# bbc/turingcodec

Hardware: AMD Instinct MI355X
Metric: encoded fps (havoc hot path, primitive-batch throughput: one picture's primitive calls per frame as whole-frame batches; (higher is better)
Workload: dtype u8; 1 GPU; 1920x1080 8-bit 4:2:0 random-access QP32 speed=medium B-frame, MEASURED call mix of the reference encoder on this clip generator (profiles/r04_reference_call_mi; calls_per_frame=3944815, launches_per_frame=49, pictures_in_flight=2, parallelism=single GPU

## Files before the change

turingcodec_amd/csrc/common.h:

```cpp
#pragma once

#include <hip/hip_runtime.h>
#include <stdint.h>

#include "../../include/havoc_mi355x.h"

namespace havoc_gpu {

constexpr int kWave = 64;

typedef uint32_t __attribute__((aligned(1))) u32u;
typedef uint32_t __attribute__((ext_vector_type(2), aligned(1))) u32x2u;
typedef uint32_t __attribute__((ext_vector_type(4), aligned(1))) u32x4u;
typedef uint32_t __attribute__((ext_vector_type(2))) u32x2;
typedef uint32_t __attribute__((ext_vector_type(4))) u32x4;
typedef short __attribute__((ext_vector_type(2))) s16x2;
typedef unsigned short __attribute__((ext_vector_type(2))) u16x2;

__device__ __forceinline__ uint32_t ld4(const void *p) { return *reinterpret_cast<const u32u *>(p); }
__device__ __forceinline__ u32x2 ld8(const void *p)
{
    u32x2u v = *reinterpret_cast<const u32x2u *>(p);
    return u32x2{v.x, v.y};
}
__device__ __forceinline__ u32x4 ld16(const void *p)
{
    u32x4u v = *reinterpret_cast<const u32x4u *>(p);
    return u32x4{v.x, v.y, v.z, v.w};
}
__device__ __forceinline__ void st4(void *p, uint32_t v) { *reinterpret_cast<u32u *>(p) = v; }
__device__ __forceinline__ void st8(void *p, u32x2 v) { *reinterpret_cast<u32x2u *>(p) = u32x2u{v.x, v.y}; }
__device__ __forceinline__ void st16(void *p, u32x4 v) { *reinterpret_cast<u32x4u *>(p) = u32x4u{v.x, v.y, v.z, v.w}; }

__device__ __forceinline__ int wave_sum(int v)
{
    v += __builtin_amdgcn_update_dpp(0, v, 0x111, 0xf, 0xf, true);
    v += __builtin_amdgcn_update_dpp(0, v, 0x112, 0xf, 0xf, true);
    v += __builtin_amdgcn_update_dpp(0, v, 0x114, 0xf, 0xe, true);
    v += __builtin_amdgcn_update_dpp(0, v, 0x118, 0xf, 0xc, true);
    v += __builtin_amdgcn_update_dpp(0, v, 0x142, 0xa, 0xf, true);
    v += __builtin_amdgcn_update_dpp(0, v, 0x143, 0xc, 0xf, true);
    return __builtin_amdgcn_readlane(v, 63);
}

__device__ __forceinline__ int row16_sum(int v)
{
    v += __builtin_amdgcn_update_dpp(0, v, 0x111, 0xf, 0xf, true);
    v += __builtin_amdgcn_update_dpp(0, v, 0x112, 0xf, 0xf, true);
    v += __builtin_amdgcn_update_dpp(0, v, 0x114, 0xf, 0xe, true);
    v += __builtin_amdgcn_update_dpp(0, v, 0x118, 0xf, 0xc, true);
    return v;
}

template <int G>
__device__ __forceinline__ int group_sum(int v)
{
#pragma unroll
    for (int o = 1; o < G; o <<= 1) v += __shfl_xor(v, o, kWave);
    return v;
}

__device__ __forceinline__ int xcd_block(int b, int nb)
{
    const int q = nb >> 3, r = nb & 7;
    const int x = b & 7, i = b >> 3;
    return x * q + min(x, r) + i;
}

__device__ __forceinline__ int clip3(int lo, int hi, int v) { return min(max(v, lo), hi); }

struct FastDiv
{
    uint32_t inv;
    int d;
    __device__ __forceinline__ explicit FastDiv(int d_) : d(d_)
    {
        const uint32_t ud = (uint32_t)d_;
        const uint32_t i0 = (uint32_t)(1048576.0f * __builtin_amdgcn_rcpf((float)d_)) - 1u;
        const uint32_t r = (1u << 20) - i0 * ud;
        inv = i0 + (r > 0u) + (r > ud) + (r > 2u * ud);
    }
    __device__ __forceinline__ int div(int i) const { return d == 1 ? i : (int)(((uint32_t)i * inv) >> 20); }
};


template <int N>
__device__ __forceinline__ void wht_inplace(int (&v)[N])
{
#pragma unroll
    for (int len = 1; len < N; len <<= 1)
#pragma unroll
        for (int i = 0; i < N; i += len << 1)
#pragma unroll
            for (int k = i; k < i + len; ++k)
            {
                const int a = v[k], b = v[k + len];
                v[k] = a + b;
                v[k + len] = a - b;
            }
}

template <int CTRL>
__device__ __forceinline__ int dpp_mov(int v)
{
    return __builtin_amdgcn_update_dpp(0, v, CTRL, 0xf, 0xf, true);
}

constexpr int kDppXor1 = 0xB1;
constexpr int kDppXor3 = 0x1B;
constexpr int kDppHalfMirror = 0x141;

template <int S, int TS>
__device__ __forceinline__ int satd_rows(int (&d)[TS], int r)
{
    wht_inplace<TS>(d);
    if (TS == 8)
    {
        const int s4 = (r & 4) ? -1 : 1;
#pragma unroll
        for (int k = 0; k < TS; ++k) d[k] = dpp_mov<kDppHalfMirror>(d[k]) + s4 * d[k];
    }
    const int s2 = (r & 2) ? -1 : 1, s1 = (r & 1) ? -1 : 1;
#pragma unroll
    for (int k = 0; k < TS; ++k) d[k] = dpp_mov<kDppXor3>(d[k]) + s2 * d[k];
    int sum = 0;
#pragma unroll
    for (int k = 0; k < TS; ++k) sum += abs(dpp_mov<kDppXor1>(d[k]) + s1 * d[k]);
    sum += dpp_mov<kDppXor1>(sum);
    sum += dpp_mov<kDppXor3>(sum);
    if (TS == 8) sum += dpp_mov<kDppHalfMirror>(sum);
    sum = (sum + TS / 4) / (TS / 2);
    if (S == 2) sum >>= 2;
    return r == 0 ? sum : 0;
}

__device__ __forceinline__ uint32_t pk_add(uint32_t a, uint32_t b)
{
    return __builtin_bit_cast(uint32_t, __builtin_bit_cast(s16x2, a) + __builtin_bit_cast(s16x2, b));
}
__device__ __forceinline__ uint32_t pk_sub(uint32_t a, uint32_t b)
{
    return __builtin_bit_cast(uint32_t, __builtin_bit_cast(s16x2, a) - __builtin_bit_cast(s16x2, b));
}
__device__ __forceinline__ uint32_t pk_bfly(uint32_t v)
{
    const u16x2 t = __builtin_bit_cast(u16x2, __builtin_amdgcn_alignbit(v, v, 16));
    const u16x2 sgn = {1, 0xffff};
    return __builtin_bit_cast(uint32_t, __builtin_bit_cast(u16x2, v) * sgn + t);
}
__device__ __forceinline__ uint32_t pk_abs_acc(uint32_t v, uint32_t acc)
{
    return __builtin_amdgcn_sad_u16(v ^ 0x80008000u, 0x80008000u, acc);
}

template <int TS>
__device__ __forceinline__ int satd_rows_pk(uint32_t (&p)[TS / 2], int r)
{
#pragma unroll
    for (int k = 0; k < TS / 2; ++k) p[k] = pk_bfly(p[k]);
#pragma unroll
    for (int len = 1; len < TS / 2; len <<= 1)
#pragma unroll
        for (int i = 0; i < TS / 2; i += len << 1)
#pragma unroll
            for (int k = i; k < i + len; ++k)
            {
                const uint32_t a = p[k], b = p[k + len];
                p[k] = pk_add(a, b);
                p[k + len] = pk_sub(a, b);
            }
    const s16x2 one = {1, 1}, neg = {-1, -1};
    if (TS == 8)
    {
        const s16x2 s4 = (r & 4) ? neg : one;
#pragma unroll
        for (int k = 0; k < TS / 2; ++k)
            p[k] = __builtin_bit_cast(uint32_t, __builtin_bit_cast(s16x2, p[k]) * s4 + __builtin_bit_cast(s16x2, (uint32_t)dpp_mov<kDppHalfMirror>((int)p[k])));
    }
    const s16x2 s2 = (r & 2) ? neg : one, s1 = (r & 1) ? neg : one;
#pragma unroll
    for (int k = 0; k < TS / 2; ++k)
        p[k] = __builtin_bit_cast(uint32_t, __builtin_bit_cast(s16x2, p[k]) * s2 + __builtin_bit_cast(s16x2, (uint32_t)dpp_mov<kDppXor3>((int)p[k])));
    uint32_t sum = 0;
#pragma unroll
    for (int k = 0; k < TS / 2; ++k)
        sum = pk_abs_acc(__builtin_bit_cast(uint32_t, __builtin_bit_cast(s16x2, p[k]) * s1 + __builtin_bit_cast(s16x2, (uint32_t)dpp_mov<kDppXor1>((int)p[k]))), sum);
    int t = (int)sum;
    t += dpp_mov<kDppXor1>(t);
    t += dpp_mov<kDppXor3>(t);
    if (TS == 8) t += dpp_mov<kDppHalfMirror>(t);
    t = (t + TS / 4) / (TS / 2);
    return r == 0 ? t : 0;
}

__device__ __forceinline__ int satd_tile8_pk(uint32_t (&d)[8][4])
{
#pragma unroll
    for (int r = 0; r < 8; ++r)
    {
        const uint32_t a0 = pk_add(d[r][0], d[r][1]), a1 = pk_sub(d[r][0], d[r][1]), a2 = pk_add(d[r][2], d[r][3]), a3 = pk_sub(d[r][2], d[r][3]);
        d[r][0] = pk_add(a0, a2); d[r][2] = pk_sub(a0, a2);
        d[r][1] = pk_add(a1, a3); d[r][3] = pk_sub(a1, a3);
    }
#pragma unroll
    for (int len = 1; len < 8; len <<= 1)
#pragma unroll
        for (int i = 0; i < 8; i += len << 1)
#pragma unroll
            for (int r = i; r < i + len; ++r)
#pragma unroll
                for (int k = 0; k < 4; ++k)
                {
                    const uint32_t a = d[r][k], b = d[r + len][k];
                    d[r][k] = pk_add(a, b);
                    d[r + len][k] = pk_sub(a, b);
                }
    uint32_t sum = 0;
#pragma unroll
    for (int r = 0; r < 8; ++r)
#pragma unroll
        for (int k = 0; k < 4; ++k) sum = pk_abs_acc(pk_bfly(d[r][k]), sum);
    return (int)((sum + 2) >> 2);
}

__device__ __forceinline__ int satd_tile8_pk16(uint32_t (&d)[8][4])
{
#pragma unroll
    for (int r = 0; r < 8; ++r)
    {
        const uint32_t a0 = pk_add(d[r][0], d[r][1]), a1 = pk_sub(d[r][0], d[r][1]), a2 = pk_add(d[r][2], d[r][3]), a3 = pk_sub(d[r][2], d[r][3]);
        d[r][0] = pk_add(a0, a2); d[r][2] = pk_sub(a0, a2);
        d[r][1] = pk_add(a1, a3); d[r][3] = pk_sub(a1, a3);
    }
#pragma unroll
    for (int len = 1; len < 8; len <<= 1)
#pragma unroll
        for (int i = 0; i < 8; i += len << 1)
#pragma unroll
            for (int r = i; r < i + len; ++r)
#pragma unroll
                for (int k = 0; k < 4; ++k)
                {
                    const uint32_t a = d[r][k], b = d[r + len][k];
                    d[r][k] = pk_add(a, b);
                    d[r + len][k] = pk_sub(a, b);
                }
    uint32_t X = 0, Y = 0;
#pragma unroll
    for (int r = 0; r < 8; ++r)
#pragma unroll
        for (int k = 0; k < 4; ++k)
        {
            const s16x2 v = __builtin_bit_cast(s16x2, d[r][k]);
            const uint32_t mag = __builtin_bit_cast(uint32_t, __builtin_elementwise_max(v, (s16x2){0, 0} - v));
            X = __builtin_amdgcn_sad_u16(mag, 0u, X);
            Y = __builtin_amdgcn_sad_u16(mag, __builtin_amdgcn_alignbit(mag, mag, 16), Y);
        }
    const uint32_t sum = X + (Y >> 1);
    return (int)(((sum + 2) >> 2) >> 2);
}


__host__ __device__ constexpr int angle_of(int mode)
{
    const int d = mode < 18 ? mode - 10 : mode - 26;
    const int mag = (int)((0x2069544d245080ull >> (6 * (d < 0 ? -d : d))) & 63);
    return (mode < 18) == (d < 0) ? mag : -mag;
}
__host__ __device__ constexpr int inv_angle_of(int mode)
{
    const int i = (mode < 18 ? mode - 10 : 26 - mode) - 1;
    const unsigned long long lo = 4096ull | (1638ull << 13) | (910ull << 26) | (630ull << 39);
    const unsigned long long hi = 482ull | (390ull << 13) | (315ull << 26) | (256ull << 39);
    return -(int)(((i < 4 ? lo : hi) >> (13 * (i & 3))) & 0x1fff);
}


typedef uint32_t __attribute__((ext_vector_type(4), aligned(2))) u32x4h;
typedef uint32_t __attribute__((ext_vector_type(2), aligned(2))) u32x2h;

template <int TS>
__device__ __forceinline__ void ld_pairs(const uint16_t *q, uint32_t (&o)[TS / 2])
{
    if constexpr (TS == 8)
    {
        const u32x4h v = *reinterpret_cast<const u32x4h *>(q);
        o[0] = v.x; o[1] = v.y; o[2] = v.z; o[3] = v.w;
    }
    else
    {
        const u32x2h v = *reinterpret_cast<const u32x2h *>(q);
        o[0] = v.x; o[1] = v.y;
    }
}

__device__ __forceinline__ uint32_t pk_mad_u16(uint32_t a, uint32_t b, uint32_t c)
{
    uint32_t d;
    asm("v_pk_mad_u16 %0, %1, %2, %3" : "=v"(d) : "v"(a), "v"(b), "v"(c));
    return d;
}
__device__ __forceinline__ uint32_t pk_lerp(uint32_t a, uint32_t b, uint32_t w0, uint32_t w1)
{
    const u16x2 five = {5, 5};
    const uint32_t t = pk_mad_u16(b, w1, pk_mad_u16(a, w0, 0x00100010u));
    return __builtin_bit_cast(uint32_t, __builtin_bit_cast(u16x2, t) >> five);
}

template <int S> struct Sample;
template <> struct Sample<1> { typedef uint8_t T; };
template <> struct Sample<2> { typedef uint16_t T; };

template <int S>
__device__ __forceinline__ uint32_t ssd_dword(uint32_t a, uint32_t b, uint32_t acc)
{
    if (S == 1)
    {
        acc = __builtin_amdgcn_udot4(a, a, acc, false);
        acc = __builtin_amdgcn_udot4(b, b, acc, false);
        const uint32_t ab = __builtin_amdgcn_udot4(a, b, 0u, false);
        return acc - 2u * ab;
    }
    const u16x2 va = __builtin_bit_cast(u16x2, a), vb = __builtin_bit_cast(u16x2, b);
    acc = __builtin_amdgcn_udot2(va, va, acc, false);
    acc = __builtin_amdgcn_udot2(vb, vb, acc, false);
    const uint32_t ab = __builtin_amdgcn_udot2(va, vb, 0u, false);
    return acc - 2u * ab;
}

}
```

turingcodec_amd/csrc/kernels_tu_fused.hip:

```cpp
#include "common.h"

#include <cstdlib>
#include "transform_basis.h"
#include "launch.h"
#include "rdoq_work.h"

namespace havoc_gpu {

template <int S, int N>
__device__ __forceinline__ void load_sample_row(const char *p, uint32_t (&row)[N / 2])
{
    if (S == 1)
    {
        uint32_t b[N / 4];
        if (N == 4) b[0] = ld4(p);
        else if (N == 8)
        {
            const u32x2 v = ld8(p);
            b[0] = v.x; b[1] = v.y;
        }
        else
        {
#pragma unroll
            for (int q = 0; q < N / 16; ++q)
            {
                const u32x4 v = ld16(p + 16 * q);
                b[4 * q] = v.x; b[4 * q + 1] = v.y; b[4 * q + 2] = v.z; b[4 * q + 3] = v.w;
            }
        }
#pragma unroll
        for (int q = 0; q < N / 4; ++q)
        {
            row[2 * q] = __builtin_amdgcn_perm(0u, b[q], 0x0c010c00u);
            row[2 * q + 1] = __builtin_amdgcn_perm(0u, b[q], 0x0c030c02u);
        }
    }
    else
    {
        if (N == 4)
        {
            const u32x2 v = ld8(p);
            row[0] = v.x; row[1] = v.y;
        }
        else
        {
#pragma unroll
            for (int q = 0; q < N / 8; ++q)
            {
                const u32x4 v = ld16(p + 16 * q);
                row[4 * q] = v.x; row[4 * q + 1] = v.y; row[4 * q + 2] = v.z; row[4 * q + 3] = v.w;
            }
        }
    }
}

template <int N>
__device__ __forceinline__ void store_staged_row(int16_t *g, const int16_t *p)
{
    if constexpr (N == 4) st8(g, *reinterpret_cast<const u32x2 *>(p));
    else st16(g, *reinterpret_cast<const u32x4 *>(p));
}

template <int S, int LOG2, int TR, bool SCAN = false>
__global__ __launch_bounds__(64) void k_tu_forward(int16_t *__restrict__ coeffs, const char *__restrict__ src, long stride_src,
                                                   const char *__restrict__ pred, long stride_pred, const int32_t *__restrict__ jobs, int njobs,
                                                   int bitDepth, const RdoqJob *__restrict__ rjobs = nullptr, int16_t *__restrict__ levels = nullptr,
                                                   RdoqWork *__restrict__ work = nullptr)
{
    constexpr int N = 1 << LOG2, TPW = 64 / N, LS = N + 2;
    __shared__ __attribute__((aligned(16))) int16_t lds[TPW][N * LS];
    const int t = threadIdx.x / N, r = threadIdx.x % N;
    const int job = xcd_block(blockIdx.x, gridDim.x) * TPW + t;
    const bool live = job < njobs;
    const int32_t *j = jobs + (long)(live ? job : 0) * 4;
    const int shift1 = LOG2 - 1 + bitDepth - 8, shift2 = LOG2 + 6;

    uint32_t row[N / 2], prow[N / 2];
    load_sample_row<S, N>(src + ((long)j[1] + (long)r * stride_src) * S, row);
    load_sample_row<S, N>(pred + ((long)j[2] + (long)r * stride_pred) * S, prow);
#pragma unroll
    for (int p = 0; p < N / 2; ++p) row[p] = pk_sub(row[p], prow[p]);
    int o[N];
    basis_times_row<N, TR, false, true>(row, 1 << (shift1 - 1), o);
#pragma unroll
    for (int k = 0; k < N; ++k) lds[t][k * LS + r] = (int16_t)(o[k] >> shift1);
    __syncthreads();
#pragma unroll
    for (int p = 0; p < N / 2; ++p) row[p] = *reinterpret_cast<const uint32_t *>(&lds[t][r * LS + 2 * p]);
    basis_times_row<N, TR, false>(row, 1 << (shift2 - 1), o);
    if (SCAN)
    {
        constexpr int GW = N / 4;
        const RdoqJob rj = rjobs[live ? job : 0];
        uint32_t thr[3];
        rdoqThresholds(rj.quant_scale, rj.quant_shift, thr);
        uint32_t lo = 0, hi = 0;
        uint64_t mask[3] = {0, 0, 0};
#pragma unroll
        for (int gy = 0; gy < GW; ++gy)
        {
            uint32_t big = 0;
#pragma unroll
            for (int k = 4 * gy; k < 4 * gy + 4; ++k)
            {
                const int c = (int16_t)(o[k] >> shift2);
                big = max(big, (uint32_t)abs(c));
                const uint32_t sq = (uint32_t)(c * c);
                lo += sq & 0xffffu;
                hi += sq >> 16;
            }
            big = max(big, (uint32_t)__shfl_xor((int)big, 1, kWave));
            big = max(big, (uint32_t)__shfl_xor((int)big, 2, kWave));
#pragma unroll
            for (int m = 0; m < 3; ++m)
            {
                const uint64_t b = __ballot(live && (r & 3) == 0 && big >= thr[m]) >> (t * N);
                uint32_t f = 0;
#pragma unroll
                for (int gx = 0; gx < GW; ++gx) f |= (uint32_t)((b >> (4 * gx)) & 1) << gx;
                mask[m] |= (uint64_t)f << (gy * GW);
            }
        }
        const int slo = group_sum<N>((int)lo), shi = group_sum<N>((int)hi);
        if (live)
        {
            int16_t *z = levels + rj.dst_off + r * N;
#pragma unroll
            for (int q = 0; q < N / 4; ++q) st8(z + 4 * q, u32x2{0, 0});
            if (r == 0)
            {
                RdoqInfo *info = reinterpret_cast<RdoqInfo *>(reinterpret_cast<char *>(work) + rdoqInfoOffset());
                RdoqInfo v;
                v.mask = mask[0];
                v.mask2 = mask[1];
                v.mask3 = mask[2];
                v.sumSq = ((int64_t)shi << 16) + slo;
                info[job] = v;
            }
        }
    }
    if constexpr (N <= 8)
    {
        __syncthreads();
#pragma unroll
        for (int k = 0; k < N; ++k) lds[t][k * N + r] = (int16_t)(o[k] >> shift2);
        __syncthreads();
        if (!live) return;
        store_staged_row<N>(coeffs + j[0] + r * N, &lds[t][r * N]);
    }
    else
    {
        if (!live) return;
        int16_t *c = coeffs + j[0] + r;
#pragma unroll
        for (int k = 0; k < N; ++k) c[k * N] = (int16_t)(o[k] >> shift2);
    }
}

template <int S, int LOG2, int TR>
__global__ __launch_bounds__(64) void k_tu_reconstruct(char *rec, long stride_rec, const char *pred, long stride_pred, const char *__restrict__ src,
                                                       long stride_src, const int16_t *__restrict__ levels, const int32_t *__restrict__ jobs,
                                                       int njobs, int bitDepth, int scale, int shift, uint32_t *__restrict__ ssd)
{
    typedef typename Sample<S>::T T;
    constexpr int N = 1 << LOG2, TPW = 64 / N, LS = N + 2;
    __shared__ int16_t lds[TPW][N * LS];
    const int t = threadIdx.x / N, r = threadIdx.x % N;
    const int job = xcd_block(blockIdx.x, gridDim.x) * TPW + t;
    const bool live = job < njobs;
    const int32_t *j = jobs + (long)(live ? job : 0) * 4;
    const int shift2 = 20 - bitDepth;
    const int dqadd = 1 << (shift - 1);

    const int16_t *c = levels + j[0] + r;
    uint32_t col[N / 2];
#pragma unroll
    for (int p = 0; p < N / 2; ++p)
    {
        const int lo = clip3(-32768, 32767, ((int)c[(2 * p) * N] * scale + dqadd) >> shift);
        const int hi = clip3(-32768, 32767, ((int)c[(2 * p + 1) * N] * scale + dqadd) >> shift);
        col[p] = ((uint32_t)lo & 0xffffu) | ((uint32_t)hi << 16);
    }
    int o[N];
    basis_times_row<N, TR, true>(col, 1 << 6, o);
#pragma unroll
    for (int k = 0; k < N; ++k) lds[t][k * LS + r] = (int16_t)clip3(-32768, 32767, o[k] >> 7);
    __syncthreads();
#pragma unroll
    for (int p = 0; p < N / 2; ++p) col[p] = *reinterpret_cast<const uint32_t *>(&lds[t][r * LS + 2 * p]);
    basis_times_row<N, TR, true>(col, 1 << (shift2 - 1), o);

    const int maxv = (1 << bitDepth) - 1;
    uint32_t prow[N / 2], srow[N / 2];
    load_sample_row<S, N>(pred + ((long)j[2] + (long)r * stride_pred) * S, prow);
    load_sample_row<S, N>(src + ((long)j[1] + (long)r * stride_src) * S, srow);
    uint32_t acc = 0;
    int v[N];
#pragma unroll
    for (int k = 0; k < N; ++k)
    {
        const int res = clip3(-32768, 32767, o[k] >> shift2);
        const int pk = (k & 1) ? (int)(prow[k >> 1] >> 16) : (int)(prow[k >> 1] & 0xffff);
        const int sk = (k & 1) ? (int)(srow[k >> 1] >> 16) : (int)(srow[k >> 1] & 0xffff);
        v[k] = clip3(0, maxv, pk + res);
        const int d = sk - v[k];
        acc += (uint32_t)(d * d);
    }
    if (live)
    {
        T *q = reinterpret_cast<T *>(rec) + j[3] + (long)r * stride_rec;
        if (S == 1)
        {
#pragma unroll
            for (int k = 0; k < N; k += 4) st4(q + k, (uint32_t)v[k] | ((uint32_t)v[k + 1] << 8) | ((uint32_t)v[k + 2] << 16) | ((uint32_t)v[k + 3] << 24));
        }
        else
        {
#pragma unroll
            for (int k = 0; k < N; k += 2) st4(q + k, (uint32_t)v[k] | ((uint32_t)v[k + 1] << 16));
        }
    }
    uint32_t tot = (uint32_t)group_sum<N>((int)acc);
    if (S == 2) tot >>= 4;
    if (live && r == 0) ssd[job] = tot;
}

template <int S, int LOG2>
__global__ __launch_bounds__(64) void k_intra_measure(int16_t *__restrict__ coeffs, int16_t *__restrict__ coeffsDct, int32_t *__restrict__ satd, char *__restrict__ rec0,
                                                      uint32_t *__restrict__ ssd0, const char *__restrict__ src, long stride_src, const char *__restrict__ pred,
                                                      long stride_pred, const int32_t *__restrict__ jobs, int njobs, int bitDepth, int withSatd)
{
    typedef typename Sample<S>::T T;
    constexpr int N = 1 << LOG2, TPW = 64 / N, LS = N + 2, TS = N >= 8 ? 8 : 4, TX = N / TS, TILES = TX * TX;
    __shared__ int16_t lds[TPW][N * LS];
    const int t = threadIdx.x / N, r = threadIdx.x % N;
    const int job = blockIdx.x * TPW + t;
    const bool live = job < njobs;
    const int32_t *j = jobs + (long)(live ? job : 0) * 4;
    const int shift1 = LOG2 - 1 + bitDepth - 8, shift2 = LOG2 + 6;

    uint32_t row[N / 2], prow[N / 2];
    load_sample_row<S, N>(src + ((long)j[1] + (long)r * stride_src) * S, row);
    load_sample_row<S, N>(pred + ((long)j[2] + (long)r * stride_pred) * S, prow);
    if (live)
    {
        const int maxv = (1 << bitDepth) - 1;
        T *q = reinterpret_cast<T *>(rec0) + j[3] + (long)r * N;
#pragma unroll
        for (int p = 0; p < N / 2; ++p)
        {
            q[2 * p] = (T)clip3(0, maxv, (int)(prow[p] & 0xffff));
            q[2 * p + 1] = (T)clip3(0, maxv, (int)(prow[p] >> 16));
        }
    }
#pragma unroll
    for (int p = 0; p < N / 2; ++p) row[p] = pk_sub(row[p], prow[p]);
    {
        uint32_t acc = 0;
#pragma unroll
        for (int p = 0; p < N / 2; ++p)
        {
            const int lo = (int16_t)(row[p] & 0xffff), hi = (int16_t)(row[p] >> 16);
            acc += (uint32_t)(lo * lo) + (uint32_t)(hi * hi);
        }
        uint32_t tot = (uint32_t)group_sum<N>((int)acc);
        if (S == 2) tot >>= 4;
        if (live && r == 0) ssd0[job] = tot;
    }
    if (withSatd)
    {
#pragma unroll
        for (int tx = 0; tx < TX; ++tx)
        {
            int c;
            if (S == 1)
            {
                uint32_t p[TS / 2];
#pragma unroll
                for (int k = 0; k < TS / 2; ++k) p[k] = row[tx * (TS / 2) + k];
                c = satd_rows_pk<TS>(p, r & (TS - 1));
            }
            else
            {
                int d[TS];
#pragma unroll
                for (int k = 0; k < TS / 2; ++k)
                {
                    d[2 * k] = (int16_t)(row[tx * (TS / 2) + k] & 0xffff);
                    d[2 * k + 1] = (int16_t)(row[tx * (TS / 2) + k] >> 16);
                }
                c = satd_rows<S, TS>(d, r & (TS - 1));
            }
            if (live && (r & (TS - 1)) == 0) satd[(long)job * TILES + (r / TS) * TX + tx] = c;
        }
    }
    uint32_t keep[N / 2];
#pragma unroll
    for (int p = 0; p < N / 2; ++p) keep[p] = row[p];
    int o[N];
    constexpr int TR = LOG2 == 2 ? 1 : 0;
    basis_times_row<N, TR, false, true>(row, 1 << (shift1 - 1), o);
#pragma unroll
    for (int k = 0; k < N; ++k) lds[t][k * LS + r] = (int16_t)(o[k] >> shift1);
    __syncthreads();
#pragma unroll
    for (int p = 0; p < N / 2; ++p) row[p] = *reinterpret_cast<const uint32_t *>(&lds[t][r * LS + 2 * p]);
    basis_times_row<N, TR, false>(row, 1 << (shift2 - 1), o);
    if (live)
    {
        int16_t *c = coeffs + j[0] + r;
#pragma unroll
        for (int k = 0; k < N; ++k) c[k * N] = (int16_t)(o[k] >> shift2);
    }
    if (LOG2 == 2)
    {
        __syncthreads();
        basis_times_row<N, 0, false, true>(keep, 1 << (shift1 - 1), o);
#pragma unroll
        for (int k = 0; k < N; ++k) lds[t][k * LS + r] = (int16_t)(o[k] >> shift1);
        __syncthreads();
#pragma unroll
        for (int p = 0; p < N / 2; ++p) row[p] = *reinterpret_cast<const uint32_t *>(&lds[t][r * LS + 2 * p]);
        basis_times_row<N, 0, false>(row, 1 << (shift2 - 1), o);
        if (live)
        {
            int16_t *c = coeffsDct + j[0] + r;
#pragma unroll
            for (int k = 0; k < N; ++k) c[k * N] = (int16_t)(o[k] >> shift2);
        }
    }
}

hipError_t launch_intra_measure(hipStream_t st, int S, int bd, int log2, int16_t *coeffs, int16_t *coeffsDct, int32_t *satd, void *rec0, uint32_t *ssd0, const void *src,
                                long ss, const void *pred, long sp, const havoc_mi355x_tu_fused_job *jobs, int n, int withSatd)
{
    if (n <= 0) return hipSuccess;
    if (log2 < 2 || log2 > 5) return hipErrorInvalidValue;
    const int tpw = 64 >> log2;
    const dim3 g((n + tpw - 1) / tpw), b(64);
    char *r0 = (char *)rec0;
    const char *s8 = (const char *)src, *p8 = (const char *)pred;
    const int32_t *j = (const int32_t *)jobs;
#define MEASURE_GO(SS, LL) hipLaunchKernelGGL((k_intra_measure<SS, LL>), g, b, 0, st, coeffs, coeffsDct, satd, r0, ssd0, s8, ss, p8, sp, j, n, bd, withSatd)
    if (S == 1) { if (log2 == 2) MEASURE_GO(1, 2); else if (log2 == 3) MEASURE_GO(1, 3); else if (log2 == 4) MEASURE_GO(1, 4); else MEASURE_GO(1, 5); }
    else { if (log2 == 2) MEASURE_GO(2, 2); else if (log2 == 3) MEASURE_GO(2, 3); else if (log2 == 4) MEASURE_GO(2, 4); else MEASURE_GO(2, 5); }
#undef MEASURE_GO
    return hipGetLastError();
}


typedef int i32x16v __attribute__((ext_vector_type(16)));
typedef int i32x4v __attribute__((ext_vector_type(4)));

struct Dct32I8 { int8_t m[32][32]; int32_t rowsum128[32]; };
constexpr Dct32I8 make_dct32_i8()
{
    Dct32I8 t{};
    for (int k = 0; k < 32; ++k)
    {
        int sum = 0;
        for (int c = 0; c < 32; ++c)
        {
            t.m[k][c] = (int8_t)basis(32, 0, k, c);
            sum += basis(32, 0, k, c);
        }
        t.rowsum128[k] = 128 * sum;
    }
    return t;
}
static __constant__ Dct32I8 c_dct32_i8 = make_dct32_i8();

__device__ __forceinline__ void mfma_dct32(const i32x4v a, const uint32_t (&v)[8], int add, int half, int (&out)[16])
{
    i32x4v bh, bl;
#pragma unroll
    for (int q = 0; q < 4; ++q)
    {
        bh[q] = (int)__builtin_amdgcn_perm(v[2 * q + 1], v[2 * q], 0x07050301u);
        bl[q] = (int)(__builtin_amdgcn_perm(v[2 * q + 1], v[2 * q], 0x06040200u) ^ 0x80808080u);
    }
    i32x16v ch, cl;
#pragma unroll
    for (int reg = 0; reg < 16; ++reg)
    {
        ch[reg] = 0;
        cl[reg] = add + c_dct32_i8.rowsum128[(reg & 3) + 8 * (reg >> 2) + 4 * half];
    }
    ch = __builtin_amdgcn_mfma_i32_32x32x32_i8(a, bh, ch, 0, 0, 0);
    cl = __builtin_amdgcn_mfma_i32_32x32x32_i8(a, bl, cl, 0, 0, 0);
#pragma unroll
    for (int reg = 0; reg < 16; ++reg) out[reg] = (int)(((uint32_t)ch[reg] << 8) + (uint32_t)cl[reg]);
}

template <bool SCAN>
__global__ __launch_bounds__(64) void k_tu_forward_mfma32(int16_t *__restrict__ coeffs, const char *__restrict__ src, long stride_src, const char *__restrict__ pred,
                                                          long stride_pred, const int32_t *__restrict__ jobs, int njobs, const RdoqJob *__restrict__ rjobs = nullptr,
                                                          int16_t *__restrict__ levels = nullptr, RdoqWork *__restrict__ work = nullptr)
{
    constexpr int LS = 40;
    __shared__ __attribute__((aligned(16))) int16_t lds[32 * LS];
    const int job = xcd_block(blockIdx.x, gridDim.x);
    if (job >= njobs) return;
    const int32_t *j = jobs + (long)job * 4;
    const int lane = threadIdx.x, y = lane & 31, half = lane >> 5;
    const i32x4v a = *reinterpret_cast<const i32x4v *>(&c_dct32_i8.m[y][16 * half]);
    uint32_t r[8];
    {
        const u32x4 s4 = ld16(src + (long)j[1] + (long)y * stride_src + 16 * half), p4 = ld16(pred + (long)j[2] + (long)y * stride_pred + 16 * half);
        const uint32_t sw[4] = {s4.x, s4.y, s4.z, s4.w}, pw[4] = {p4.x, p4.y, p4.z, p4.w};
#pragma unroll
        for (int q = 0; q < 4; ++q)
        {
            r[2 * q] = pk_sub(__builtin_amdgcn_perm(0u, sw[q], 0x0c010c00u), __builtin_amdgcn_perm(0u, pw[q], 0x0c010c00u));
            r[2 * q + 1] = pk_sub(__builtin_amdgcn_perm(0u, sw[q], 0x0c030c02u), __builtin_amdgcn_perm(0u, pw[q], 0x0c030c02u));
        }
    }
    int t[16];
    mfma_dct32(a, r, 8, half, t);
#pragma unroll
    for (int reg = 0; reg < 16; ++reg) lds[((reg & 3) + 8 * (reg >> 2) + 4 * half) * LS + y] = (int16_t)(t[reg] >> 4);
    __syncthreads();
    uint32_t v[8];
    {
        const u32x4 q0 = *reinterpret_cast<const u32x4 *>(&lds[y * LS + 16 * half]), q1 = *reinterpret_cast<const u32x4 *>(&lds[y * LS + 16 * half + 8]);
        v[0] = q0.x; v[1] = q0.y; v[2] = q0.z; v[3] = q0.w; v[4] = q1.x; v[5] = q1.y; v[6] = q1.z; v[7] = q1.w;
    }
    int o[16];
    mfma_dct32(a, v, 1024, half, o);
    int16_t *c = coeffs + j[0] + y;
#pragma unroll
    for (int reg = 0; reg < 16; ++reg) c[((reg & 3) + 8 * (reg >> 2) + 4 * half) * 32] = (int16_t)(o[reg] >> 11);
    if (SCAN)
    {
        const RdoqJob rj = rjobs[job];
        uint32_t thr[3];
        rdoqThresholds(rj.quant_scale, rj.quant_shift, thr);
        uint32_t lo = 0, hi = 0;
        uint64_t mask[3] = {0, 0, 0};
#pragma unroll
        for (int q = 0; q < 4; ++q)
        {
            uint32_t big = 0;
#pragma unroll
            for (int k = 0; k < 4; ++k)
            {
                const int cf = (int16_t)(o[4 * q + k] >> 11);
                big = max(big, (uint32_t)abs(cf));
                const uint32_t sq = (uint32_t)(cf * cf);
                lo += sq & 0xffffu;
                hi += sq >> 16;
            }
            big = max(big, (uint32_t)__shfl_xor((int)big, 1, kWave));
            big = max(big, (uint32_t)__shfl_xor((int)big, 2, kWave));
#pragma unroll
            for (int m = 0; m < 3; ++m)
            {
                uint64_t b = __ballot((y & 3) == 0 && big >= thr[m]);
                b = (b | b >> 3) & 0x0303030303030303ull;
                b = (b | b >> 6) & 0x000f000f000f000full;
                b = (b | b >> 12) & 0x000000ff000000ffull;
                mask[m] |= (b & 0xffu) << (16 * q) | (b >> 32) << (16 * q + 8);
            }
        }
        const int slo = wave_sum((int)lo), shi = wave_sum((int)hi);
        int16_t *z = levels + rj.dst_off + lane * 16;
        st8(z, u32x2{0, 0}); st8(z + 4, u32x2{0, 0}); st8(z + 8, u32x2{0, 0}); st8(z + 12, u32x2{0, 0});
        if (lane == 0)
        {
            RdoqInfo *info = reinterpret_cast<RdoqInfo *>(reinterpret_cast<char *>(work) + rdoqInfoOffset());
            RdoqInfo w;
            w.mask = mask[0];
            w.mask2 = mask[1];
            w.mask3 = mask[2];
            w.sumSq = ((int64_t)shi << 16) + slo;
            info[job] = w;
        }
    }
}

static bool mfmaForward()
{
    static const bool on = !(getenv("HAVOC_TU_MFMA") && atoi(getenv("HAVOC_TU_MFMA")) == 0);
    return on;
}

template <int S, int LOG2, int TR>
static void go_fwd(hipStream_t st, int16_t *co, const char *src, long ss, const char *pred, long sp, const int32_t *j, int n, int bd)
{
    constexpr int TPW = 64 >> LOG2;
    hipLaunchKernelGGL((k_tu_forward<S, LOG2, TR>), dim3((n + TPW - 1) / TPW), dim3(64), 0, st, co, src, ss, pred, sp, j, n, bd);
}

template <int S>
static hipError_t launch_fwd_s(hipStream_t st, int bd, int log2, int tr, int16_t *co, const char *src, long ss, const char *pred, long sp,
                               const int32_t *j, int n)
{
    if (tr)
    {
        if (log2 != 2) return hipErrorInvalidValue;
        go_fwd<S, 2, 1>(st, co, src, ss, pred, sp, j, n, bd);
    }
    else
        switch (log2)
        {
        case 2: go_fwd<S, 2, 0>(st, co, src, ss, pred, sp, j, n, bd); break;
        case 3: go_fwd<S, 3, 0>(st, co, src, ss, pred, sp, j, n, bd); break;
        case 4: go_fwd<S, 4, 0>(st, co, src, ss, pred, sp, j, n, bd); break;
        case 5:
            if (S == 1 && bd == 8 && mfmaForward()) hipLaunchKernelGGL((k_tu_forward_mfma32<false>), dim3(n), dim3(64), 0, st, co, src, ss, pred, sp, j, n);
            else go_fwd<S, 5, 0>(st, co, src, ss, pred, sp, j, n, bd);
            break;
        default: return hipErrorInvalidValue;
        }
    return hipGetLastError();
}

hipError_t launch_tu_forward_scan(hipStream_t st, int S, int bd, int log2, int16_t *coeffs, const void *src, long ss, const void *pred, long sp,
                                  const havoc_mi355x_tu_fused_job *jobs, int n, const RdoqJob *rj, int16_t *levels, void *workspace)
{
    if (n <= 0) return hipSuccess;
    if (log2 != 4 && log2 != 5) return hipErrorInvalidValue;
    const char *s8 = (const char *)src, *p8 = (const char *)pred;
    const int32_t *j = (const int32_t *)jobs;
    RdoqWork *w = (RdoqWork *)workspace;
    const int tpw = 64 >> log2;
    const dim3 g((n + tpw - 1) / tpw), b(64);
    if (S == 1 && log2 == 4) hipLaunchKernelGGL((k_tu_forward<1, 4, 0, true>), g, b, 0, st, coeffs, s8, ss, p8, sp, j, n, bd, rj, levels, w);
    else if (S == 1 && bd == 8 && mfmaForward()) hipLaunchKernelGGL((k_tu_forward_mfma32<true>), dim3(n), b, 0, st, coeffs, s8, ss, p8, sp, j, n, rj, levels, w);
    else if (S == 1) hipLaunchKernelGGL((k_tu_forward<1, 5, 0, true>), g, b, 0, st, coeffs, s8, ss, p8, sp, j, n, bd, rj, levels, w);
    else if (log2 == 4) hipLaunchKernelGGL((k_tu_forward<2, 4, 0, true>), g, b, 0, st, coeffs, s8, ss, p8, sp, j, n, bd, rj, levels, w);
    else hipLaunchKernelGGL((k_tu_forward<2, 5, 0, true>), g, b, 0, st, coeffs, s8, ss, p8, sp, j, n, bd, rj, levels, w);
    return hipGetLastError();
}

hipError_t launch_tu_forward(hipStream_t st, int S, int bd, int log2, int tr, int16_t *coeffs, const void *src, long ss, const void *pred, long sp,
                             const havoc_mi355x_tu_fused_job *jobs, int n)
{
    if (n <= 0) return hipSuccess;
    return S == 1 ? launch_fwd_s<1>(st, bd, log2, tr, coeffs, (const char *)src, ss, (const char *)pred, sp, (const int32_t *)jobs, n)
                  : launch_fwd_s<2>(st, bd, log2, tr, coeffs, (const char *)src, ss, (const char *)pred, sp, (const int32_t *)jobs, n);
}

template <int S, int LOG2, int TR>
static void go_rec(hipStream_t st, char *rec, long sr, const char *pred, long sp, const char *src, long ss, const int16_t *lv, const int32_t *j, int n,
                   int bd, int scale, int shift, uint32_t *ssd)
{
    constexpr int TPW = 64 >> LOG2;
    hipLaunchKernelGGL((k_tu_reconstruct<S, LOG2, TR>), dim3((n + TPW - 1) / TPW), dim3(64), 0, st, rec, sr, pred, sp, src, ss, lv, j, n, bd, scale,
                       shift, ssd);
}

template <int S>
static hipError_t launch_rec_s(hipStream_t st, int bd, int log2, int tr, int scale, int shift, char *rec, long sr, const char *pred, long sp,
                               const char *src, long ss, const int16_t *lv, const int32_t *j, int n, uint32_t *ssd)
{
    if (tr)
    {
        if (log2 != 2) return hipErrorInvalidValue;
        go_rec<S, 2, 1>(st, rec, sr, pred, sp, src, ss, lv, j, n, bd, scale, shift, ssd);
    }
    else
        switch (log2)
        {
        case 2: go_rec<S, 2, 0>(st, rec, sr, pred, sp, src, ss, lv, j, n, bd, scale, shift, ssd); break;
        case 3: go_rec<S, 3, 0>(st, rec, sr, pred, sp, src, ss, lv, j, n, bd, scale, shift, ssd); break;
        case 4: go_rec<S, 4, 0>(st, rec, sr, pred, sp, src, ss, lv, j, n, bd, scale, shift, ssd); break;
        case 5: go_rec<S, 5, 0>(st, rec, sr, pred, sp, src, ss, lv, j, n, bd, scale, shift, ssd); break;
        default: return hipErrorInvalidValue;
        }
    return hipGetLastError();
}

hipError_t launch_tu_reconstruct(hipStream_t st, int S, int bd, int log2, int tr, int scale, int shift, void *rec, long sr, const void *pred, long sp,
                                 const void *src, long ss, const int16_t *levels, const havoc_mi355x_tu_fused_job *jobs, int n, uint32_t *ssd)
{
    if (n <= 0) return hipSuccess;
    return S == 1 ? launch_rec_s<1>(st, bd, log2, tr, scale, shift, (char *)rec, sr, (const char *)pred, sp, (const char *)src, ss, levels,
                                    (const int32_t *)jobs, n, ssd)
                  : launch_rec_s<2>(st, bd, log2, tr, scale, shift, (char *)rec, sr, (const char *)pred, sp, (const char *)src, ss, levels,
                                    (const int32_t *)jobs, n, ssd);
}

}
```

Before: 1646 frames/s.

## Trim VALU work in TU forward scan and reconstruct with packed 16-bit ops

The forward-transform RDOQ scan now packs coefficient pairs, takes magnitudes and squares with packed/dot ops, reduces the group max with DPP moves instead of shuffles, and builds significance masks with one ballot plus bit compression per threshold. The reconstruct kernel uses packed saturating conversion, add and clip for the residual path, mul24 for dequantisation when the scale fits in 24 bits, and dot-product SSD accumulation over packed output words. The aim is fewer VALU instructions, 32-bit multiplies and cross-lane ops per wavefront. Profiling scripts for instruction classes and traces are added, and the mask layout change carries a risk of subtle bit-order bugs.

```diff
diff --git a/profiles/tu_diet/issue_classes.py b/profiles/tu_diet/issue_classes.py
--- /dev/null
+++ b/profiles/tu_diet/issue_classes.py
@@ -0,0 +1,83 @@
+#!/usr/bin/env python3
+import re
+import sys
+
+STEP = [
+    ("k_tu_forward", (1, 2, 0, 0), 2965),
+    ("k_tu_forward", (1, 2, 1, 0), 8331),
+    ("k_tu_forward", (1, 3, 0, 0), 11100),
+    ("k_tu_forward", (1, 4, 0, 1), 13704),
+    ("k_tu_forward_mfma32", (1,), 14735),
+    ("k_tu_reconstruct", (1, 2, 1), 8331),
+    ("k_tu_reconstruct", (1, 3, 0), 11100),
+    ("k_tu_reconstruct", (1, 4, 0), 13704),
+    ("k_tu_reconstruct", (1, 5, 0), 7368),
+]
+CLASSES = ("dot/mfma", "pk16", "mul_lo/mad64", "other VALU", "SALU", "SMEM", "LDS", "VMEM")
+SLOW = ("v_mul_lo_u32", "v_mul_hi_u32", "v_mul_hi_i32", "v_mad_u64_u32", "v_mad_i64_i32")
+NOT_ISSUED_WORK = ("s_waitcnt", "s_nop", "s_endpgm", "s_barrier", "s_code_end")
+
+
+def classify(op):
+    if op.startswith(("v_dot", "v_mfma")):
+        return "dot/mfma"
+    if op.startswith("v_pk_") or op.startswith("v_cvt_pk_i16") or op.startswith("v_cvt_pk_u16"):
+        return "pk16"
+    if op.startswith(SLOW):
+        return "mul_lo/mad64"
+    if op.startswith("v_"):
+        return "other VALU"
+    if op.startswith(("s_load", "s_buffer_load")):
+        return "SMEM"
+    if op.startswith("s_"):
+        return None if op.startswith(NOT_ISSUED_WORK) else "SALU"
+    if op.startswith("ds_"):
+        return "LDS"
+    if op.startswith(("global_", "flat_", "buffer_", "scratch_")):
+        return "VMEM"
+    return None
+
+
+def instances(listing):
+    out, cur = {}, None
+    for line in open(listing):
+        m = re.match(r"^(_ZN9havoc_gpu\d+(k_tu_\w+?)I((?:L[ib]\d+E)+)E\w*):", line)
+        if m:
+            cur = out.setdefault((m.group(2), tuple(int(a) for a in re.findall(r"L[ib](\d+)E", m.group(3)))), dict.fromkeys(CLASSES, 0))
+            continue
+        if cur is None:
+            continue
+        if line.startswith(".Lfunc_end"):
+            cur = None
+            continue
+        m = re.match(r"^\s+([a-z][a-z0-9_]+)", line)
+        if m:
+            c = classify(m.group(1))
+            if c:
+                cur[c] += 1
+    return out
+
+
+def main():
+    args = [a for a in sys.argv[1:] if a != "--all"]
+    inst = instances(args[0])
+    label = args[1] if len(args) > 1 else args[0]
+    print(f"# {label}: instructions per wavefront by class | the same times the wavefronts of the step's large launch, in thousands")
+    print(f"{'kernel':34s} {'wavefronts':>10s} " + " ".join(f"{c:>12s}" for c in CLASSES) + f" {'VALU':>6s}")
+    rows = [(k, a, w) for k, a, w in STEP] if "--all" not in sys.argv else [(k, a, 0) for k, a in sorted(inst)]
+    for kernel, targs, waves in rows:
+        keys = [key for key in inst if key[0] == kernel and key[1][:len(targs)] == targs and all(key[1][len(targs):])]
+        if not keys:
+            print(f"{kernel}<{','.join(map(str, targs))}>: not in the listing")
+            continue
+        key = min(keys, key=lambda k: len(k[1]))
+        c = inst[key]
+        valu = c["dot/mfma"] + c["pk16"] + c["mul_lo/mad64"] + c["other VALU"]
+        name = f"{kernel}<{','.join(map(str, key[1]))}>"
+        print(f"{name:34s} {waves:10d} " + " ".join(f"{c[x]:12d}" for x in CLASSES) + f" {valu:6d}")
+        if waves:
+            print(f"{'':34s} {'x waves, k':>10s} " + " ".join(f"{c[x] * waves / 1000:12.0f}" for x in CLASSES) + f" {valu * waves / 1000:6.0f}")
+
+
+if __name__ == "__main__":
+    main()
diff --git a/profiles/tu_diet/trace_table.py b/profiles/tu_diet/trace_table.py
--- /dev/null
+++ b/profiles/tu_diet/trace_table.py
@@ -0,0 +1,67 @@
+#!/usr/bin/env python3
+import csv
+import glob
+import os
+import statistics
+import sys
+from collections import defaultdict
+
+KERNELS = ("k_tu_forward", "k_tu_reconstruct", "k_ssd<")
+
+
+def short(name):
+    return name.replace("void ", "").replace("havoc_gpu::", "").split("(")[0]
+
+
+def rows_of(d, suffix):
+    for f in sorted(glob.glob(os.path.join(d, "**", "*" + suffix), recursive=True)):
+        yield from csv.DictReader(open(f))
+
+
+def by_launch(dispatches, steps):
+    dispatches = sorted(dispatches)
+    per = len(dispatches) // steps if len(dispatches) % steps == 0 else len(dispatches)
+    out = defaultdict(list)
+    for i, (_, v) in enumerate(dispatches):
+        out[i % per].append(v)
+    return out
+
+
+def main():
+    mode, d, steps = sys.argv[1], sys.argv[2], int(sys.argv[3])
+    w = csv.writer(sys.stdout, lineterminator="\n")
+    if mode == "trace":
+        seen = defaultdict(list)
+        for r in rows_of(d, "kernel_trace.csv"):
+            k = short(r["Kernel_Name"])
+            if any(p in k for p in KERNELS):
+                waves = int(r["Grid_Size_X"]) * int(r.get("Grid_Size_Y", 1) or 1) * int(r.get("Grid_Size_Z", 1) or 1) // 64
+                seen[k].append((int(r["Dispatch_Id"]), (int(r["End_Timestamp"]) - int(r["Start_Timestamp"]), waves, r.get("VGPR_Count", ""), r.get("LDS_Block_Size", ""))))
+        w.writerow(["kernel", "launch", "wavefronts", "vgprs", "lds_bytes", "steps", "min_ns", "median_ns", "max_ns"])
+        total = 0.0
+        for k in sorted(seen):
+            for launch, vals in sorted(by_launch(seen[k], steps).items()):
+                ns = [v[0] for v in vals]
+                w.writerow([k, launch, vals[0][1], vals[0][2], vals[0][3], len(ns), min(ns), int(statistics.median(ns)), max(ns)])
+                if k.startswith("k_tu_"):
+                    total += statistics.median(ns)
+        w.writerow(["all k_tu_* launches of a step (sum of medians)", "", "", "", "", "", "", int(total), ""])
+    else:
+        seen = defaultdict(lambda: defaultdict(lambda: defaultdict(float)))
+        grid = {}
+        for r in rows_of(d, "counter_collection.csv"):
+            k = short(r["Kernel_Name"])
+            if any(p in k for p in KERNELS):
+                seen[k][r["Counter_Name"]][int(r["Dispatch_Id"])] += float(r["Counter_Value"])
+                grid[k, int(r["Dispatch_Id"])] = int(r["Grid_Size"]) // 64
+        names = sorted({c for k in seen for c in seen[k]})
+        w.writerow(["kernel", "launch", "wavefronts"] + names)
+        for k in sorted(seen):
+            cols = {c: by_launch(list(seen[k][c].items()), steps) for c in names}
+            ids = by_launch([(i, i) for i in seen[k][names[0]]], steps)
+            for launch in sorted(ids):
+                w.writerow([k, launch, grid[k, ids[launch][0]]] + [int(statistics.mean(cols[c][launch])) if cols[c].get(launch) else "" for c in names])
+
+
+if __name__ == "__main__":
+    main()
diff --git a/turingcodec_amd/csrc/common.h b/turingcodec_amd/csrc/common.h
--- a/turingcodec_amd/csrc/common.h
+++ b/turingcodec_amd/csrc/common.h
@@ -260,6 +260,39 @@
     return (int)(((sum + 2) >> 2) >> 2);
 }
 
+__device__ __forceinline__ uint32_t pk_sat_i16(int lo, int hi)
+{
+    return __builtin_bit_cast(uint32_t, __builtin_amdgcn_cvt_pk_i16(lo, hi));
+}
+__device__ __forceinline__ uint32_t pk_add_sat(uint32_t a, uint32_t b)
+{
+    return __builtin_bit_cast(uint32_t, __builtin_elementwise_add_sat(__builtin_bit_cast(s16x2, a), __builtin_bit_cast(s16x2, b)));
+}
+__device__ __forceinline__ uint32_t pk_clip(uint32_t v, uint32_t lo, uint32_t hi)
+{
+    return __builtin_bit_cast(uint32_t, __builtin_elementwise_min(__builtin_elementwise_max(__builtin_bit_cast(s16x2, v), __builtin_bit_cast(s16x2, lo)),
+                                                                  __builtin_bit_cast(s16x2, hi)));
+}
+__device__ __forceinline__ uint32_t pk_mag(uint32_t v)
+{
+    const s16x2 s = __builtin_bit_cast(s16x2, v);
+    return __builtin_bit_cast(uint32_t, __builtin_elementwise_max(s, (s16x2){0, 0} - s));
+}
+__device__ __forceinline__ uint32_t pk_max_u(uint32_t a, uint32_t b)
+{
+    return __builtin_bit_cast(uint32_t, __builtin_elementwise_max(__builtin_bit_cast(u16x2, a), __builtin_bit_cast(u16x2, b)));
+}
+
+template <int FIELD>
+__device__ __forceinline__ uint64_t quad_ballot_compress(uint64_t b)
+{
+    static_assert(FIELD == 16 || FIELD == 32, "a field is 16 or 32 lanes");
+    b = (b | b >> 3) & 0x0303030303030303ull;
+    b = (b | b >> 6) & 0x000f000f000f000full;
+    if (FIELD == 32) b = (b | b >> 12) & 0x000000ff000000ffull;
+    return b;
+}
+
 
 __host__ __device__ constexpr int angle_of(int mode)
 {
@@ -312,19 +345,27 @@
 template <> struct Sample<2> { typedef uint16_t T; };
 
 template <int S>
+__device__ __forceinline__ void ssd_dword_acc(uint32_t a, uint32_t b, uint32_t &sq, uint32_t &cross)
+{
+    if (S == 1)
+    {
+        sq = __builtin_amdgcn_udot4(a, a, sq, false);
+        sq = __builtin_amdgcn_udot4(b, b, sq, false);
+        cross = __builtin_amdgcn_udot4(a, b, cross, false);
+    }
+    else
+    {
+        const u16x2 va = __builtin_bit_cast(u16x2, a), vb = __builtin_bit_cast(u16x2, b);
+        sq = __builtin_amdgcn_udot2(va, va, sq, false);
+        sq = __builtin_amdgcn_udot2(vb, vb, sq, false);
+        cross = __builtin_amdgcn_udot2(va, vb, cross, false);
+    }
+}
+template <int S>
 __device__ __forceinline__ uint32_t ssd_dword(uint32_t a, uint32_t b, uint32_t acc)
 {
-    if (S == 1)
-    {
-        acc = __builtin_amdgcn_udot4(a, a, acc, false);
-        acc = __builtin_amdgcn_udot4(b, b, acc, false);
-        const uint32_t ab = __builtin_amdgcn_udot4(a, b, 0u, false);
-        return acc - 2u * ab;
-    }
-    const u16x2 va = __builtin_bit_cast(u16x2, a), vb = __builtin_bit_cast(u16x2, b);
-    acc = __builtin_amdgcn_udot2(va, va, acc, false);
-    acc = __builtin_amdgcn_udot2(vb, vb, acc, false);
-    const uint32_t ab = __builtin_amdgcn_udot2(va, vb, 0u, false);
+    uint32_t ab = 0;
+    ssd_dword_acc<S>(a, b, acc, ab);
     return acc - 2u * ab;
 }
 
diff --git a/turingcodec_amd/csrc/kernels_tu_fused.hip b/turingcodec_amd/csrc/kernels_tu_fused.hip
--- a/turingcodec_amd/csrc/kernels_tu_fused.hip
+++ b/turingcodec_amd/csrc/kernels_tu_fused.hip
@@ -8,26 +8,31 @@
 namespace havoc_gpu {
 
 template <int S, int N>
-__device__ __forceinline__ void load_sample_row(const char *p, uint32_t (&row)[N / 2])
-{
-    if (S == 1)
-    {
-        uint32_t b[N / 4];
-        if (N == 4) b[0] = ld4(p);
-        else if (N == 8)
-        {
-            const u32x2 v = ld8(p);
-            b[0] = v.x; b[1] = v.y;
-        }
-        else
-        {
-#pragma unroll
-            for (int q = 0; q < N / 16; ++q)
-            {
-                const u32x4 v = ld16(p + 16 * q);
-                b[4 * q] = v.x; b[4 * q + 1] = v.y; b[4 * q + 2] = v.z; b[4 * q + 3] = v.w;
-            }
-        }
+__device__ __forceinline__ void load_raw_row(const char *p, uint32_t (&b)[N * S / 4])
+{
+    constexpr int B = N * S;
+    if constexpr (B == 4) b[0] = ld4(p);
+    else if constexpr (B == 8)
+    {
+        const u32x2 v = ld8(p);
+        b[0] = v.x; b[1] = v.y;
+    }
+    else
+    {
+#pragma unroll
+        for (int q = 0; q < B / 16; ++q)
+        {
+            const u32x4 v = ld16(p + 16 * q);
+            b[4 * q] = v.x; b[4 * q + 1] = v.y; b[4 * q + 2] = v.z; b[4 * q + 3] = v.w;
+        }
+    }
+}
+
+template <int S, int N>
+__device__ __forceinline__ void unpack_sample_row(const uint32_t (&b)[N * S / 4], uint32_t (&row)[N / 2])
+{
+    if constexpr (S == 1)
+    {
 #pragma unroll
         for (int q = 0; q < N / 4; ++q)
         {
@@ -37,21 +42,17 @@
     }
     else
     {
-        if (N == 4)
-        {
-            const u32x2 v = ld8(p);
-            row[0] = v.x; row[1] = v.y;
-        }
-        else
-        {
-#pragma unroll
-            for (int q = 0; q < N / 8; ++q)
-            {
-                const u32x4 v = ld16(p + 16 * q);
-                row[4 * q] = v.x; row[4 * q + 1] = v.y; row[4 * q + 2] = v.z; row[4 * q + 3] = v.w;
-            }
-        }
-    }
+#pragma unroll
+        for (int q = 0; q < N / 2; ++q) row[q] = b[q];
+    }
+}
+
+template <int S, int N>
+__device__ __forceinline__ void load_sample_row(const char *p, uint32_t (&row)[N / 2])
+{
+    uint32_t b[N * S / 4];
+    load_raw_row<S, N>(p, b);
+    unpack_sample_row<S, N>(b, row);
 }
 
 template <int N>
@@ -59,6 +60,19 @@
 {
     if constexpr (N == 4) st8(g, *reinterpret_cast<const u32x2 *>(p));
     else st16(g, *reinterpret_cast<const u32x4 *>(p));
+}
+
+__device__ __forceinline__ uint32_t scan_group(int c0, int c1, int c2, int c3, uint32_t &lo, uint32_t &hi)
+{
+    const uint32_t m0 = pk_mag(__builtin_amdgcn_perm((uint32_t)c1, (uint32_t)c0, 0x05040100u)), m1 = pk_mag(__builtin_amdgcn_perm((uint32_t)c3, (uint32_t)c2, 0x05040100u));
+    const uint32_t s0 = __builtin_amdgcn_udot2(__builtin_bit_cast(u16x2, m0), __builtin_bit_cast(u16x2, m0), 0u, false);
+    const uint32_t s1 = __builtin_amdgcn_udot2(__builtin_bit_cast(u16x2, m1), __builtin_bit_cast(u16x2, m1), 0u, false);
+    lo += (s0 & 0xffffu) + (s1 & 0xffffu);
+    hi += (s0 >> 16) + (s1 >> 16);
+    const uint32_t m = pk_max_u(m0, m1);
+    uint32_t big = max(m & 0xffffu, m >> 16);
+    big = max(big, (uint32_t)dpp_mov<kDppXor1>((int)big));
+    return max(big, (uint32_t)dpp_mov<kDppXor3>((int)big));
 }
 
 template <int S, int LOG2, int TR, bool SCAN = false>
@@ -88,39 +102,33 @@
 #pragma unroll
     for (int p = 0; p < N / 2; ++p) row[p] = *reinterpret_cast<const uint32_t *>(&lds[t][r * LS + 2 * p]);
     basis_times_row<N, TR, false>(row, 1 << (shift2 - 1), o);
-    if (SCAN)
+    if constexpr (SCAN)
     {
         constexpr int GW = N / 4;
         const RdoqJob rj = rjobs[live ? job : 0];
         uint32_t thr[3];
         rdoqThresholds(rj.quant_scale, rj.quant_shift, thr);
         uint32_t lo = 0, hi = 0;
-        uint64_t mask[3] = {0, 0, 0};
+        uint64_t acc[3][N / 16] = {};
 #pragma unroll
         for (int gy = 0; gy < GW; ++gy)
         {
-            uint32_t big = 0;
-#pragma unroll
-            for (int k = 4 * gy; k < 4 * gy + 4; ++k)
-            {
-                const int c = (int16_t)(o[k] >> shift2);
-                big = max(big, (uint32_t)abs(c));
-                const uint32_t sq = (uint32_t)(c * c);
-                lo += sq & 0xffffu;
-                hi += sq >> 16;
-            }
-            big = max(big, (uint32_t)__shfl_xor((int)big, 1, kWave));
-            big = max(big, (uint32_t)__shfl_xor((int)big, 2, kWave));
+            const uint32_t big = scan_group(o[4 * gy] >> shift2, o[4 * gy + 1] >> shift2, o[4 * gy + 2] >> shift2, o[4 * gy + 3] >> shift2, lo, hi);
 #pragma unroll
             for (int m = 0; m < 3; ++m)
             {
-                const uint64_t b = __ballot(live && (r & 3) == 0 && big >= thr[m]) >> (t * N);
-                uint32_t f = 0;
-#pragma unroll
-                for (int gx = 0; gx < GW; ++gx) f |= (uint32_t)((b >> (4 * gx)) & 1) << gx;
-                mask[m] |= (uint64_t)f << (gy * GW);
+                const uint64_t b = quad_ballot_compress<N>(__ballot(big >= thr[m]) & 0x1111111111111111ull);
+                if constexpr (N == 16) acc[m][0] |= b << (gy * GW);
+                else
+                {
+                    acc[m][0] |= (b & 0xffu) << (gy * GW);
+                    acc[m][1] |= (b >> 32) << (gy * GW);
+                }
             }
         }
+        uint64_t mask[3];
+#pragma unroll
+        for (int m = 0; m < 3; ++m) mask[m] = N == 16 ? (acc[m][0] >> (t * N)) & 0xffffu : t ? acc[m][N / 16 - 1] : acc[m][0];
         const int slo = group_sum<N>((int)lo), shi = group_sum<N>((int)hi);
         if (live)
         {
@@ -157,7 +165,7 @@
     }
 }
 
-template <int S, int LOG2, int TR>
+template <int S, int LOG2, int TR, bool MAD24>
 __global__ __launch_bounds__(64) void k_tu_reconstruct(char *rec, long stride_rec, const char *pred, long stride_pred, const char *__restrict__ src,
                                                        long stride_src, const int16_t *__restrict__ levels, const int32_t *__restrict__ jobs,
                                                        int njobs, int bitDepth, int scale, int shift, uint32_t *__restrict__ ssd)
@@ -177,50 +185,45 @@
 #pragma unroll
     for (int p = 0; p < N / 2; ++p)
     {
-        const int lo = clip3(-32768, 32767, ((int)c[(2 * p) * N] * scale + dqadd) >> shift);
-        const int hi = clip3(-32768, 32767, ((int)c[(2 * p + 1) * N] * scale + dqadd) >> shift);
-        col[p] = ((uint32_t)lo & 0xffffu) | ((uint32_t)hi << 16);
+        const int l0 = c[(2 * p) * N], l1 = c[(2 * p + 1) * N];
+        const int lo = MAD24 ? __mul24(l0, scale) + dqadd : l0 * scale + dqadd, hi = MAD24 ? __mul24(l1, scale) + dqadd : l1 * scale + dqadd;
+        col[p] = pk_sat_i16(lo >> shift, hi >> shift);
     }
     int o[N];
     basis_times_row<N, TR, true>(col, 1 << 6, o);
 #pragma unroll
-    for (int k = 0; k < N; ++k) lds[t][k * LS + r] = (int16_t)clip3(-32768, 32767, o[k] >> 7);
+    for (int k = 0; k < N; k += 2)
+    {
+        const uint32_t pair = pk_sat_i16(o[k] >> 7, o[k + 1] >> 7);
+        lds[t][k * LS + r] = (int16_t)(pair & 0xffffu);
+        lds[t][(k + 1) * LS + r] = (int16_t)(pair >> 16);
+    }
     __syncthreads();
 #pragma unroll
     for (int p = 0; p < N / 2; ++p) col[p] = *reinterpret_cast<const uint32_t *>(&lds[t][r * LS + 2 * p]);
     basis_times_row<N, TR, true>(col, 1 << (shift2 - 1), o);
 
-    const int maxv = (1 << bitDepth) - 1;
-    uint32_t prow[N / 2], srow[N / 2];
+    const uint32_t maxv = (1u << bitDepth) - 1, maxv2 = maxv | maxv << 16;
+    uint32_t prow[N / 2], sraw[N * S / 4];
     load_sample_row<S, N>(pred + ((long)j[2] + (long)r * stride_pred) * S, prow);
-    load_sample_row<S, N>(src + ((long)j[1] + (long)r * stride_src) * S, srow);
-    uint32_t acc = 0;
-    int v[N];
-#pragma unroll
-    for (int k = 0; k < N; ++k)
-    {
-        const int res = clip3(-32768, 32767, o[k] >> shift2);
-        const int pk = (k & 1) ? (int)(prow[k >> 1] >> 16) : (int)(prow[k >> 1] & 0xffff);
-        const int sk = (k & 1) ? (int)(srow[k >> 1] >> 16) : (int)(srow[k >> 1] & 0xffff);
-        v[k] = clip3(0, maxv, pk + res);
-        const int d = sk - v[k];
-        acc += (uint32_t)(d * d);
+    load_raw_row<S, N>(src + ((long)j[1] + (long)r * stride_src) * S, sraw);
+    uint32_t v[N / 2];
+#pragma unroll
+    for (int p = 0; p < N / 2; ++p) v[p] = pk_clip(pk_add_sat(prow[p], pk_sat_i16(o[2 * p] >> shift2, o[2 * p + 1] >> shift2)), 0u, maxv2);
+    uint32_t out[N * S / 4], sq = 0, cross = 0;
+#pragma unroll
+    for (int q = 0; q < N * S / 4; ++q)
+    {
+        out[q] = S == 1 ? __builtin_amdgcn_perm(v[(2 * q + 1) % (N / 2)], v[(2 * q) % (N / 2)], 0x06040200u) : v[q % (N / 2)];
+        ssd_dword_acc<S>(out[q], sraw[q], sq, cross);
     }
     if (live)
     {
         T *q = reinterpret_cast<T *>(rec) + j[3] + (long)r * stride_rec;
-        if (S == 1)
-        {
-#pragma unroll
-            for (int k = 0; k < N; k += 4) st4(q + k, (uint32_t)v[k] | ((uint32_t)v[k + 1] << 8) | ((uint32_t)v[k + 2] << 16) | ((uint32_t)v[k + 3] << 24));
-        }
-        else
-        {
-#pragma unroll
-            for (int k = 0; k < N; k += 2) st4(q + k, (uint32_t)v[k] | ((uint32_t)v[k + 1] << 16));
-        }
-    }
-    uint32_t tot = (uint32_t)group_sum<N>((int)acc);
+#pragma unroll
+        for (int k = 0; k < N * S / 4; ++k) st4(q + k * (4 / S), out[k]);
+    }
+    uint32_t tot = (uint32_t)group_sum<N>((int)(sq - 2u * cross));
     if (S == 2) tot >>= 4;
     if (live && r == 0) ssd[job] = tot;
 }
@@ -430,7 +433,7 @@
     int16_t *c = coeffs + j[0] + y;
 #pragma unroll
     for (int reg = 0; reg < 16; ++reg) c[((reg & 3) + 8 * (reg >> 2) + 4 * half) * 32] = (int16_t)(o[reg] >> 11);
-    if (SCAN)
+    if constexpr (SCAN)
     {
         const RdoqJob rj = rjobs[job];
         uint32_t thr[3];
@@ -455,10 +458,7 @@
 #pragma unroll
             for (int m = 0; m < 3; ++m)
             {
-                uint64_t b = __ballot((y & 3) == 0 && big >= thr[m]);
-                b = (b | b >> 3) & 0x0303030303030303ull;
-                b = (b | b >> 6) & 0x000f000f000f000full;
-                b = (b | b >> 12) & 0x000000ff000000ffull;
+                const uint64_t b = quad_ballot_compress<32>(__ballot((y & 3) == 0 && big >= thr[m]));
                 mask[m] |= (b & 0xffu) << (16 * q) | (b >> 32) << (16 * q + 8);
             }
         }
@@ -546,8 +546,11 @@
                    int bd, int scale, int shift, uint32_t *ssd)
 {
     constexpr int TPW = 64 >> LOG2;
-    hipLaunchKernelGGL((k_tu_reconstruct<S, LOG2, TR>), dim3((n + TPW - 1) / TPW), dim3(64), 0, st, rec, sr, pred, sp, src, ss, lv, j, n, bd, scale,
-                       shift, ssd);
+    const dim3 g((n + TPW - 1) / TPW), b(64);
+    if (scale >= -(1 << 23) && scale < (1 << 23))
+        hipLaunchKernelGGL((k_tu_reconstruct<S, LOG2, TR, true>), g, b, 0, st, rec, sr, pred, sp, src, ss, lv, j, n, bd, scale, shift, ssd);
+    else
+        hipLaunchKernelGGL((k_tu_reconstruct<S, LOG2, TR, false>), g, b, 0, st, rec, sr, pred, sp, src, ss, lv, j, n, bd, scale, shift, ssd);
 }
 
 template <int S>
```

After: 1571 frames/s. 4.6% lower.
